# HKPolyU-UAV/FLVIS

Hardware: AMD Instinct MI355X
Metric: frames/sec/node (640×480 stereo+IMU) + ATE vs CPU ref, EuRoC MH_05 (higher is better)
Workload: dtype u8/f32 LK+GFTT, f64 geometry+BA

## Files before the change

### flvis_amd/csrc/capi.cpp

```cpp
#include <cmath>
#include <cstdint>
#include <cstdio>
#include <cstring>
#include <vector>

#include "../../include/flvis_hip.h"
#include "ctx.hpp"
#include "pipeline.hpp"

using namespace flvis;

void* flvis_ctx::scratch(const std::string& name, size_t bytes, bool zero_on_alloc) {
  Buf& b = bufs[name];
  if (b.bytes >= bytes && b.p) return b.p;
  if (b.p) {
    hipStreamSynchronize(stream);
    hipFree(b.p);
    b.p = nullptr;
    b.bytes = 0;
  }
  size_t want = (bytes + 255) / 256 * 256;
  if (hipMalloc(&b.p, want) != hipSuccess) {
    b.p = nullptr;
    return nullptr;
// ... 176 lines not shown
    total += pyr.stride[l] * n_img + 256;
    total = (total + 255) / 256 * 256;
  }
  uint8_t* base = (uint8_t*)ctx->scratch(name, total + 256);
  if (!base && L > 0) return ctx->fail(FLVIS_ERR_HIP, "pyramid scratch allocation failed");
  for (int l = 1; l <= L; l++) {
    pyr.lvl[l] = img_plain(base + off[l]);
    launch_pyr_down(ctx->stream, pyr.lvl[l - 1], pyr.w[l - 1], pyr.h[l - 1], pyr.pitch[l - 1], pyr.stride[l - 1],
                    pyr.lvl[l], pyr.pitch[l], pyr.stride[l], n_img, nullptr);
  }
  return FLVIS_OK;
}

int flvis_hip_lk_track(flvis_ctx* ctx, const uint8_t* d_prev, const uint8_t* d_next, int w, int h, int n_img,
                       const float* d_prev_pts, float* d_next_pts, uint8_t* d_status, const int* d_count, int nmax,
                       int max_level, int max_iter, double eps, int use_initial_flow) {
  CHECK_CTX(ctx);
  if (!d_prev || !d_next || !d_prev_pts || !d_next_pts || !d_status || !d_count || w < 32 || h < 32 || n_img <= 0 || nmax <= 0 ||
      max_level < 0)
    return ctx->fail(FLVIS_ERR_INVALID_ARG, "lk_track: bad args");
  int L = lk_levels(w, h, 31, max_level);
  if (L >= LK_MAX_LEVELS) L = LK_MAX_LEVELS - 1;
  PyrSel pp, pn;
  int rc = build_pyramid(ctx, "lk_pyr_prev", d_prev, w, h, n_img, L, pp);
  if (rc) return rc;
  rc = build_pyramid(ctx, "lk_pyr_next", d_next, w, h, n_img, L, pn);
  if (rc) return rc;
  LKParams prm;
  prm.max_iter = max_iter < 0 ? 0 : (max_iter > 100 ? 100 : max_iter);
  double e = eps < 0 ? 0 : (eps > 10 ? 10 : eps);
  prm.eps2 = e * e;
  prm.min_eig = 1e-4f;
  prm.use_initial = use_initial_flow ? 1 : 0;
  launch_lk_track(ctx->stream, pp, pn, d_prev_pts, d_next_pts, d_status, d_count, nmax, n_img, prm, nullptr);
  CHECK_LAUNCH(ctx, "lk_track");
  return FLVIS_OK;
}

int flvis_hip_rand_seed(flvis_ctx* ctx, uint32_t seed, int32_t* d_state35, int n_sets) {
  CHECK_CTX(ctx);
  if (!d_state35 || n_sets <= 0) return ctx->fail(FLVIS_ERR_INVALID_ARG, "rand_seed: bad args");
  std::vector<int> h((size_t)35 * n_sets);
  glibc_seed(seed, h.data());
  h[34] = 0;
  for (int s = 1; s < n_sets; s++) memcpy(&h[(size_t)35 * s], h.data(), sizeof(int) * 35);
  hipError_t e = hipMemcpyAsync(d_state35, h.data(), sizeof(int) * h.size(), hipMemcpyHostToDevice, ctx->stream);
  if (e == hipSuccess) e = hipStreamSynchronize(ctx->stream);
  if (e != hipSuccess) return ctx->hip_fail(e, "rand_seed");
  return FLVIS_OK;
}

int flvis_hip_stereo_depth(flvis_ctx* ctx, const flvis_cfg* cfg, const uint8_t* d_img0, const uint8_t* d_img1, int n_sets,
                           const float* d_pt2d_plane, const float* d_pt2d_undistort, const float* d_pt3d_w, const uint8_t* d_has_depth,
                           const int* d_count, int cap, const double* h_T_c_w7, float range, int32_t* d_rand_state35, double* d_pt3d_c,
                           uint8_t* d_mask_has_3d) {
  CHECK_CTX(ctx);
  if (!cfg || !d_img0 || !d_img1 || !d_pt2d_plane || !d_pt2d_undistort || !d_pt3d_w || !d_has_depth || !d_count || !h_T_c_w7 ||
      !d_rand_state35 || !d_pt3d_c || !d_mask_has_3d || n_sets <= 0 || cap <= 0)
    return ctx->fail(FLVIS_ERR_INVALID_ARG, "stereo_depth: bad args");
  if (cfg->cam_type == CAM_DEPTH) return ctx->fail(FLVIS_ERR_CONFIG, "stereo_depth: the rig has a depth camera (recover3DPts_c_FromDepthImg), no stereo pair");
  const int w = cfg->image_width, h = cfg->image_height;
  if (w < 32 || h < 32) return ctx->fail(FLVIS_ERR_CONFIG, "stereo_depth: image too small");
  if (cfg->P0[0] == 0.0 || cfg->P0[5] == 0.0 || cfg->P1[0] == 0.0)
    return ctx->fail(FLVIS_ERR_CONFIG, "stereo_depth: the configuration is not finalised (flvis_config_finalize: P0 / P1 are empty)");
  flvis_sd_cam cam;
  memcpy(cam.K1, cfg->cam1_intrinsics, 32);
  memcpy(cam.D1, cfg->cam1_distortion, 32);
  memcpy(cam.R1, cfg->R1, 72);
// ... 152 lines not shown
```

### flvis_amd/csrc/ctx.hpp

```cpp
#pragma once
#include <hip/hip_runtime.h>

#include <map>
#include <memory>
#include <string>

#include "img_kernels.hpp"

namespace flvis {
struct Pipeline;
}

struct flvis_ctx {
  int device = 0;
  hipStream_t stream = nullptr;
  bool own_stream = false;
  std::string err;

  struct Buf {
    void* p = nullptr;
    size_t bytes = 0;
  };
  std::map<std::string, Buf> bufs;
  flvis::Pipeline* pipe = nullptr;
  int voc_nodes = 0, voc_words = 0, voc_depth = 0;
  std::string orb_pattern;

  void* scratch(const std::string& name, size_t bytes, bool zero_on_alloc = false);
  int fail(int code, const std::string& msg) {
    err = msg;
    return code;
  }
  int hip_fail(hipError_t e, const char* what) {
    err = std::string(what) + ": " + hipGetErrorString(e);
    return -3;
  }
};

static inline int align_up(int v, int a) { return (v + a - 1) / a * a; }
```

### flvis_amd/csrc/img_kernels.hpp

```cpp
#pragma once
#include <hip/hip_runtime.h>
#include <stdint.h>

namespace flvis {

struct KJoin {
  const long long* wait[2];
  long long wait_seq[2];
  long long* sig;
  long long sig_seq;
  unsigned* sig_cnt;
  long long* err;
  const long long* post;
  long long post_seq;
};


struct ImgSel {
  const uint8_t* b[2];
  const int* cur;
  int flip;
  const uint8_t* const* ind;
  __device__ const uint8_t* ptr(int s, size_t stride) const {
    if (ind) return *ind + (size_t)s * stride;
    int k = cur ? (cur[s] ^ flip) : 0;
    return b[k] + (size_t)s * stride;
  }
};
static inline ImgSel img_plain(const uint8_t* p) { return ImgSel{{p, p}, nullptr, 0, nullptr}; }
static inline ImgSel img_indirect(const uint8_t* const* slot) { return ImgSel{{nullptr, nullptr}, nullptr, 0, slot}; }

constexpr int LK_MAX_LEVELS = 6;
struct PyrSel {
  ImgSel lvl[LK_MAX_LEVELS];
  int w[LK_MAX_LEVELS], h[LK_MAX_LEVELS], pitch[LK_MAX_LEVELS];
  size_t stride[LK_MAX_LEVELS];
  int levels;
  int bx[LK_MAX_LEVELS] = {}, by[LK_MAX_LEVELS] = {};
};
constexpr int LK_BORDER_X = 32, LK_BORDER_Y = 24;

struct LKParams {
  int max_iter;
  double eps2;
  float min_eig;
  int use_initial;
  unsigned long long* stats = nullptr;
  unsigned long long* stats_tc = nullptr;
  uint32_t* tc = nullptr;
  int tc_mode = 0, tc_cap = 0, tc_stride = 0;
  const int* tc_slot = nullptr;
  const long long* tc_tag = nullptr;
  int order = 0;
  int dbg_slot = 0;
};
int lk_tc_slot_dwords(int levels);
__device__ inline int lk_tc_lookup(const uint32_t* tc, int tc_cap, int tc_stride, int s, int slot, float px, float py, long long tag) {
  if (!tc || slot < 0 || slot >= tc_cap) return -1;
  const uint32_t* h = tc + ((size_t)s * tc_cap + slot) * tc_stride;
  if (h[0] != __float_as_uint(px) || h[1] != __float_as_uint(py) || *reinterpret_cast<const long long*>(h + 2) != tag) return -1;
  return slot | (int)((h[4] & 0x7fffu) << 16);
}

struct DemParams {
  int regionWidth, regionHeight, boundary_dis;
  unsigned max_region_feature_num;
};

struct GfttScratch {
  unsigned* maxenc;
  int* nkeys;
  unsigned long long* keys;
  int cap;
};

hipError_t img_kernels_init();
void launch_equalize_hist(hipStream_t st, ImgSel src, ImgSel dst, int w, int h, int spitch, int dpitch, size_t sstride,
                          size_t dstride, int S, unsigned* hist, uint8_t* lut, const int* active);
void launch_bgr_to_gray(hipStream_t st, const uint8_t* src, int channels, uint8_t* dst, size_t npixels);
void launch_copy_image(hipStream_t st, ImgSel src, ImgSel dst, int w, int h, int spitch, int dpitch, size_t sstride,
                       size_t dstride, int S, const int* active);
// ... 42 lines not shown
```

### flvis_amd/csrc/lk_kernel.hip

```cpp
#include "dev_common.hpp"
#include "img_kernels.hpp"

namespace flvis {

constexpr int LK_WIN = 31;
constexpr int LK_PS = 40;
constexpr int LK_PROWS = 34;
constexpr int LK_RM = 4;
constexpr int LK_RS = 52;
constexpr int LK_RROWS = 33 + 2 * LK_RM;
constexpr int LK_TC_HDR = 64;
constexpr int LK_TC_LVL = 64 * 24;

typedef short lk_s2 __attribute__((ext_vector_type(2)));
typedef __attribute__((address_space(1))) uint32_t lk_gu32;
typedef uint32_t lk_u4 __attribute__((ext_vector_type(4)));
__device__ __forceinline__ lk_s2 lk_as_s2(uint32_t v) { return __builtin_bit_cast(lk_s2, v); }

__device__ __forceinline__ bool lk_load_patch(const uint8_t* __restrict__ img, int w, int h, int pitch, int bx, int by, int X0, int Y0,
                                              int nrows, uint8_t* patch) {
  if (X0 >= -bx && Y0 >= -by && X0 + 39 < w + bx && Y0 + nrows <= h + by) {
    const lk_gu32* const base = (const lk_gu32*)(img + (ptrdiff_t)Y0 * pitch + (X0 & ~3));
    const int sh = X0 & 3;
    int r = (int)threadIdx.x / 9, k = (int)threadIdx.x - 9 * r;
// ... 58 lines not shown
    constexpr int N = LK_RROWS * 13, T = (N + 63) / 64;
    uint32_t v[T];
#pragma unroll
    for (int t = 0; t < T; t++) {
      const bool on = 64 * (t + 1) <= N || (int)threadIdx.x + 64 * t < N;
      v[t] = *(const lk_gu32*)(base + (on ? off : 0u));
      k += 12;
      const bool wrap = k >= 13;
      k = wrap ? k - 13 : k;
      off += (unsigned)(4 * pitch + 48) + (wrap ? (unsigned)(pitch - 52) : 0u);
    }
#pragma unroll
    for (int t = 0; t < T; t++) asm volatile("" : "+v"(v[t]));
#pragma unroll
    for (int t = 0; t < T; t++)
      if (64 * (t + 1) <= N || (int)threadIdx.x + 64 * t < N) *reinterpret_cast<uint32_t*>(region + 4 * ((int)threadIdx.x + 64 * t)) = v[t];
    return false;
  }
  for (int i = threadIdx.x; i < LK_RROWS * 13; i += 64) {
    int r = i / 13, k = i - r * 13;
    int Y = Y0 + r, X = X0 + 4 * k;
    uint32_t v;
    if (Y >= 0 && Y < h && X >= 0 && X + 3 < w) {
      v = *reinterpret_cast<const uint32_t*>(img + (size_t)Y * pitch + X);
    } else {
      const uint8_t* row = img + (size_t)reflect101c(Y, h) * pitch;
      uint32_t b0 = row[reflect101c(X, w)], b1 = row[reflect101c(X + 1, w)], b2 = row[reflect101c(X + 2, w)],
               b3 = row[reflect101c(X + 3, w)];
      v = b0 | (b1 << 8) | (b2 << 16) | (b3 << 24);
    }
    *reinterpret_cast<uint32_t*>(region + r * LK_RS + 4 * k) = v;
  }
  return true;
}

#define LK_PAIR(D, K)                                                                                              \
  ((((K)&3) == 3) ? __builtin_amdgcn_perm((D)[((K) >> 2) + 1], (D)[(K) >> 2], 0x0c040c03u)                         \
                  : __builtin_amdgcn_perm(0u, (D)[(K) >> 2], 0x0c000c00u | (uint32_t)((K)&3) | ((uint32_t)(((K)&3) + 1) << 16)))

__device__ __forceinline__ int lk_dot2_bias(lk_s2 a, lk_s2 b, int bias_uniform) {
  int r;
  asm("v_dot2_i32_i16 %0, %1, %2, %3" : "=v"(r) : "v"(a), "v"(b), "s"(bias_uniform));
  return r;
}
__device__ __forceinline__ void lk_wave_sum2_f32(int v1, int v2, float& f1, float& f2) {
  int a = v1 & 0xffff, b = v1 >> 16, c = v2 & 0xffff, d = v2 >> 16;
#define LK_STEP4(CTRL, RM)                                           \
  {                                                                  \
    const int ta = __builtin_amdgcn_update_dpp(0, a, CTRL, RM, 0xf, false); \
    const int tb = __builtin_amdgcn_update_dpp(0, b, CTRL, RM, 0xf, false); \
    const int tc = __builtin_amdgcn_update_dpp(0, c, CTRL, RM, 0xf, false); \
    const int td = __builtin_amdgcn_update_dpp(0, d, CTRL, RM, 0xf, false); \
    a += ta, b += tb, c += tc, d += td;                              \
  }
  LK_STEP4(0xB1, 0xf)
  LK_STEP4(0x4E, 0xf)
  LK_STEP4(0x141, 0xf)
  LK_STEP4(0x140, 0xf)
  LK_STEP4(0x142, 0xa)
  LK_STEP4(0x143, 0xc)
#undef LK_STEP4
  const float g1 = (float)__builtin_fma((double)b, 65536.0, (double)a), g2 = (float)__builtin_fma((double)d, 65536.0, (double)c);
  f1 = __builtin_bit_cast(float, __builtin_amdgcn_readlane(__builtin_bit_cast(int, g1), 63));
  f2 = __builtin_bit_cast(float, __builtin_amdgcn_readlane(__builtin_bit_cast(int, g2), 63));
}

// ... 183 lines not shown
#ifdef FLVIS_LK_UTIL
__device__ unsigned long long g_lk_wt[3][8][32768][2];
#define LK_UTIL_BEGIN const unsigned long long lk_t0_ = wall_clock64(); const unsigned lk_widx_ = (blockIdx.y * gridDim.x + blockIdx.x) & 32767u;
#define LK_UTIL_END(ROLE)                                                              \
  if (threadIdx.x == 0) {                                                              \
    unsigned long long* u_ = g_lk_wt[(ROLE) % 3][prm.dbg_slot & 7][lk_widx_];          \
    u_[0] = lk_t0_;                                                                    \
    u_[1] = wall_clock64();                                                            \
  }
#else
#define LK_UTIL_BEGIN
#define LK_UTIL_END(ROLE)
#endif
template <int ROLE>
__device__ __forceinline__ void lk_track_body(const PyrSel& prev, const PyrSel& next, const float* __restrict__ prev_pts,
                                              float* __restrict__ next_pts, uint8_t* __restrict__ status,
                                              const int* __restrict__ count, int nmax, const LKParams& prm,
                                              const int* __restrict__ active) {
  int s = blockIdx.y, bx = blockIdx.x;
  {
    const int G = gridDim.x, N = G * gridDim.y;
    if ((N & 7) == 0) {
      const int L = bx + G * s;
      const int Lp = (L & 7) * (N >> 3) + (L >> 3);
      s = Lp / G;
      bx = Lp - s * G;
    }
  }
  if (active && !active[s]) return;
  int n = count[s];
  if (n > nmax) n = nmax;
  if (bx >= n) return;
  LK_UTIL_BEGIN
  __shared__ __attribute__((aligned(16))) uint8_t patch[LK_RROWS * LK_RS + 12];
  const int lane = threadIdx.x;
  int kc_prev = 0, kc_next = 0;
#pragma unroll
  for (int l = LK_MAX_LEVELS - 1; l >= 0; l--) {
    if (l <= prev.levels && prev.lvl[l].cur) kc_prev = prev.lvl[l].cur[s];
    if (l <= next.levels && next.lvl[l].cur) kc_next = next.lvl[l].cur[s];
  }
  const uint8_t* const ind_prev0 = prev.lvl[0].ind ? *prev.lvl[0].ind : nullptr;
  const uint8_t* const ind_next0 = next.lvl[0].ind ? *next.lvl[0].ind : nullptr;
  const int r = lane >> 1;
  const int c0 = (lane & 1) * 16;
  const int W_BITS = 14;
  double eps2 = prm.eps2;
  if (ROLE == 1 || ROLE == 4) asm volatile("" : "+v"(eps2));
  const float FLT_SCALE = 1.f / (1 << 20);
  const float halfWin = (LK_WIN - 1) * 0.5f;

  for (int pb = bx; pb < n; pb += gridDim.x) {
    const int p = prm.order == 1 ? n - 1 - pb : pb;
    const size_t pi = ((size_t)s * nmax + p) * 2;
    const float ppx0 = prev_pts[pi], ppy0 = prev_pts[pi + 1];
    float nx = next_pts[pi], ny = next_pts[pi + 1];
    int st = 1;
    uint32_t* tc_ptr = nullptr;
    bool tc_store = false, tc_hit = false;
    uint32_t tc_mask = 0;
    if (ROLE == 2 && prm.tc_mode == 1) {
      if (p < prm.tc_cap) {
        tc_store = true;
        tc_ptr = prm.tc + ((size_t)s * prm.tc_cap + p) * prm.tc_stride;
      }
    } else if ((ROLE == 1 && prm.tc_mode == 2) || (ROLE == 4 && prm.tc_mode == 3)) {
      const int code = __builtin_amdgcn_readfirstlane(prm.tc_slot[(size_t)s * nmax + p]);
      if (code >= 0 && (code & 0xffff) < prm.tc_cap) {
        tc_ptr = prm.tc + ((size_t)s * prm.tc_cap + (code & 0xffff)) * prm.tc_stride;
        tc_hit = true;
        tc_mask = (uint32_t)code >> 16;
      } else if (ROLE == 4 && code <= -2 && -code - 2 < prm.tc_cap) {
        tc_ptr = prm.tc + ((size_t)s * prm.tc_cap + (-code - 2)) * prm.tc_stride;
        tc_store = true;
      }
    }
    lk_u4 pq[6] = {};
    int pq_level = -1;
    for (int level = prev.levels; level >= 0; level--) {
      const float sc = (float)(1. / (1 << level));
      float ppx = ppx0 * sc, ppy = ppy0 * sc;
      float npx, npy;
      if (level == prev.levels) {
        if (prm.use_initial) {
          npx = nx * sc;
          npy = ny * sc;
        } else {
          npx = ppx;
          npy = ppy;
        }
      } else {
        npx = nx * 2.f;
        npy = ny * 2.f;
      }
      nx = npx;
      ny = npy;
      const int W = prev.w[level], H = prev.h[level];
      ppx -= halfWin;
      ppy -= halfWin;
      const int ipx = (int)floorf(ppx), ipy = (int)floorf(ppy);
      if (ipx < -LK_WIN || ipx >= W || ipy < -LK_WIN || ipy >= H) {
        if (level == 0) st = 0;
        continue;
      }
      float a = ppx - (float)ipx, b = ppy - (float)ipy;
      int iw00 = __float2int_rn((1.f - a) * (1.f - b) * (float)(1 << W_BITS));
      int iw01 = __float2int_rn(a * (1.f - b) * (float)(1 << W_BITS));
      int iw10 = __float2int_rn((1.f - a) * b * (float)(1 << W_BITS));
      int iw11 = (1 << W_BITS) - iw00 - iw01 - iw10;

      lk_s2 tI[8], tX[8], tY[8];
      long long iA11, iA12, iA22;
      const bool cached = (ROLE == 1 || ROLE == 4) && tc_hit && ((tc_mask >> level) & 1u);
      constexpr bool kEarlyRegion = (ROLE == 1 || ROLE == 4) && FLVIS_LK_EARLY_REGION;
      int JW = 0, JH = 0;
      const uint8_t* Jimg = nullptr;
      if (kEarlyRegion) {
        JW = next.w[level], JH = next.h[level];
        Jimg = lk_level_ptr(next, level, s, kc_next, ind_next0);
      }
      bool region_ok = false;
      int RX0 = 0, RY0 = 0;
      if (cached) {
        if (prm.stats_tc && lane == 0) atomicAdd(&prm.stats_tc[0], 1ull);
        if (pq_level != level) {
          const lk_u4* src = reinterpret_cast<const lk_u4*>(tc_ptr + LK_TC_HDR + (size_t)level * LK_TC_LVL) + lane;
#pragma unroll
          for (int k = 0; k < 6; k++) pq[k] = __builtin_nontemporal_load(src + 64 * k);
        }
        if (kEarlyRegion) {
        {
          const int einx = (int)floorf(npx - halfWin), einy = (int)floorf(npy - halfWin);
          if (!(einx < -LK_WIN || einx >= JW || einy < -LK_WIN || einy >= JH)) {
            RX0 = (einx - LK_RM) & ~3;
            RY0 = einy - LK_RM;
            __syncthreads();
            const bool slow = lk_load_region(Jimg, JW, JH, next.pitch[level], next.bx[level], next.by[level], RX0, RY0, patch);
            __syncthreads();
            if (prm.stats_tc && slow && lane == 0) atomicAdd(&prm.stats_tc[2], 1ull);
            region_ok = true;
          }
        }
        }
        lk_u4 q[6];
#pragma unroll
        for (int k = 0; k < 6; k++) q[k] = pq[k];
        pq_level = -1;
        iA11 = (long long)(((unsigned long long)(uint32_t)__builtin_amdgcn_readlane((int)q[0].y, 63) << 32) | (uint32_t)__builtin_amdgcn_readlane((int)q[0].x, 63));
        iA12 = (long long)(((unsigned long long)(uint32_t)__builtin_amdgcn_readlane((int)q[0].w, 63) << 32) | (uint32_t)__builtin_amdgcn_readlane((int)q[0].z, 63));
        iA22 = (long long)(((unsigned long long)(uint32_t)__builtin_amdgcn_readlane((int)q[1].y, 63) << 32) | (uint32_t)__builtin_amdgcn_readlane((int)q[1].x, 63));
#pragma unroll
        for (int k = 0; k < 2; k++) {
          tI[4 * k + 0] = lk_as_s2(q[k].x); tI[4 * k + 1] = lk_as_s2(q[k].y);
          tI[4 * k + 2] = lk_as_s2(q[k].z); tI[4 * k + 3] = lk_as_s2(q[k].w);
          tX[4 * k + 0] = lk_as_s2(q[2 + k].x); tX[4 * k + 1] = lk_as_s2(q[2 + k].y);
          tX[4 * k + 2] = lk_as_s2(q[2 + k].z); tX[4 * k + 3] = lk_as_s2(q[2 + k].w);
          tY[4 * k + 0] = lk_as_s2(q[4 + k].x); tY[4 * k + 1] = lk_as_s2(q[4 + k].y);
          tY[4 * k + 2] = lk_as_s2(q[4 + k].z); tY[4 * k + 3] = lk_as_s2(q[4 + k].w);
        }
      } else if (ROLE == 1 || ROLE == 4) {
        LKTmpl T;
        lk_template_level_cold(lk_level_ptr(prev, level, s, kc_prev, ind_prev0), W, H, prev.pitch[level], prev.bx[level], prev.by[level], ipx, ipy, iw00,
                               iw01, iw10, iw11, patch, lane, &T);
#pragma unroll
        for (int k = 0; k < 8; k++) {
          tI[k] = lk_as_s2(T.w[k]);
          tX[k] = lk_as_s2(T.w[8 + k]);
          tY[k] = lk_as_s2(T.w[16 + k]);
        }
        iA11 = T.a11;
        iA12 = T.a12;
        iA22 = T.a22;
        if (ROLE == 4 && tc_store) {
          lk_tc_store_level(tc_ptr, level, lane, tI, tX, tY, iA11, iA12, iA22);
          tc_mask |= 1u << level;
        }
      } else {
        const bool slow = lk_template_level(lk_level_ptr(prev, level, s, kc_prev, ind_prev0), W, H, prev.pitch[level], prev.bx[level], prev.by[level], ipx,
                                            ipy, iw00, iw01, iw10, iw11, patch, lane, tI, tX, tY, iA11, iA12, iA22);
        if (prm.stats_tc && slow && lane == 0) atomicAdd(&prm.stats_tc[1], 1ull);
#ifndef FLVIS_LK_NO_TC_STORE
        if (ROLE == 2 && tc_store) {
          lk_tc_store_level(tc_ptr, level, lane, tI, tX, tY, iA11, iA12, iA22);
          tc_mask |= 1u << level;
        }
#endif
      }
      const float A11 = (float)iA11 * FLT_SCALE, A12 = (float)iA12 * FLT_SCALE, A22 = (float)iA22 * FLT_SCALE;
      float D = A11 * A22 - A12 * A12;
      const float minEig = __fdiv_rn(A22 + A11 - sqrtf((A11 - A22) * (A11 - A22) + 4.f * A12 * A12),
                                     (float)(2 * LK_WIN * LK_WIN));
      if (minEig < prm.min_eig || D < 1.1920929e-07f) {
        if (level == 0) st = 0;
        continue;
      }
      D = __fdiv_rn(1.f, D);
      npx -= halfWin;
      npy -= halfWin;
      float pdx = 0.f, pdy = 0.f;
      if (!kEarlyRegion) {
        JW = next.w[level], JH = next.h[level];
        Jimg = lk_level_ptr(next, level, s, kc_next, ind_next0);
      }
      int iters_run = 0;
      for (int j = 0; j < prm.max_iter; j++) {
        iters_run = j + 1;
        const int inx = (int)floorf(npx), iny = (int)floorf(npy);
        if (inx < -LK_WIN || inx >= JW || iny < -LK_WIN || iny >= JH) {
          if (level == 0) st = 0;
          break;
        }
        a = npx - (float)inx;
        b = npy - (float)iny;
        iw00 = __float2int_rn((1.f - a) * (1.f - b) * (float)(1 << W_BITS));
        iw01 = __float2int_rn(a * (1.f - b) * (float)(1 << W_BITS));
        iw10 = __float2int_rn((1.f - a) * b * (float)(1 << W_BITS));
        iw11 = (1 << W_BITS) - iw00 - iw01 - iw10;
        if (!region_ok || inx < RX0 || inx - RX0 > 15 || iny < RY0 || iny - RY0 > 2 * LK_RM) {
          RX0 = (inx - LK_RM) & ~3;
          RY0 = iny - LK_RM;
          __syncthreads();
          const bool slow = lk_load_region(Jimg, JW, JH, next.pitch[level], next.bx[level], next.by[level], RX0, RY0, patch);
          __syncthreads();
          if (prm.stats_tc && slow && lane == 0) atomicAdd(&prm.stats_tc[2], 1ull);
          region_ok = true;
        }
        int b1 = 0, b2 = 0;
        if (r < LK_WIN) {
          const int bx = inx - RX0 + c0, sh = bx & 3;
          const uint8_t* rp = patch + (iny - RY0 + r) * LK_RS + (bx & ~3);
          uint32_t e[2][5];
#pragma unroll
          for (int q = 0; q < 2; q++) {
            uint32_t dd[6];
#pragma unroll
            for (int k = 0; k < 6; k++) dd[k] = *reinterpret_cast<const uint32_t*>(rp + q * LK_RS + 4 * k);
#pragma unroll
            for (int k = 0; k < 5; k++) e[q][k] = __builtin_amdgcn_alignbyte(dd[k + 1], dd[k], sh);
          }
          const lk_s2 wT = lk_s2{(short)iw00, (short)iw01}, wB = lk_s2{(short)iw10, (short)iw11};
#pragma unroll
          for (int c2 = 0; c2 < 8; c2++) {
            int iv[2];
#pragma unroll
            for (int hh = 0; hh < 2; hh++) {
              const int c = 2 * c2 + hh;
              const uint32_t pt = LK_PAIR(e[0], c), pb = LK_PAIR(e[1], c);
              int acc = lk_dot2_bias(__builtin_bit_cast(lk_s2, pt), wT, 1 << (W_BITS - 5 - 1));
              acc = __builtin_amdgcn_sdot2(__builtin_bit_cast(lk_s2, pb), wB, acc, false);
              iv[hh] = acc >> (W_BITS - 5);
            }
            const lk_s2 ivp = __builtin_bit_cast(lk_s2, __builtin_amdgcn_perm((uint32_t)iv[1], (uint32_t)iv[0], 0x05040100u));
            const lk_s2 diff = ivp - tI[c2];
            b1 = __builtin_amdgcn_sdot2(diff, tX[c2], b1, false);
            b2 = __builtin_amdgcn_sdot2(diff, tY[c2], b2, false);
          }
        }
        float sb1, sb2;
        lk_wave_sum2_f32(b1, b2, sb1, sb2);
        const float fb1 = sb1 * FLT_SCALE, fb2 = sb2 * FLT_SCALE;
        const float ddx = (A12 * fb2 - A22 * fb1) * D;
        const float ddy = (A12 * fb1 - A11 * fb2) * D;
        npx += ddx;
        npy += ddy;
        nx = npx + halfWin;
        ny = npy + halfWin;
        if ((double)ddx * (double)ddx + (double)ddy * (double)ddy <= eps2) break;
        if (j > 0 && fabs((double)(ddx + pdx)) < 0.01 && fabs((double)(ddy + pdy)) < 0.01) {
          nx -= ddx * 0.5f;
          ny -= ddy * 0.5f;
          break;
        }
        pdx = ddx;
        pdy = ddy;
      }
      if (prm.stats && lane == 0) {
        atomicAdd(&prm.stats[2 * level], (unsigned long long)iters_run);
        atomicAdd(&prm.stats[2 * level + 1], 1ull);
      }
      if (st && level == 0) {
        const float fx = nx - halfWin, fy = ny - halfWin;
        const int inx = (int)floorf(fx), iny = (int)floorf(fy);
        if (inx < -LK_WIN || inx >= JW || iny < -LK_WIN || iny >= JH) st = 0;
      }
    }
    if (lane == 0) {
      next_pts[pi] = nx;
      next_pts[pi + 1] = ny;
      status[(size_t)s * nmax + p] = (uint8_t)st;
      if ((ROLE == 2 || ROLE == 4) && tc_store) {
        tc_ptr[0] = __float_as_uint(ppx0);
        tc_ptr[1] = __float_as_uint(ppy0);
        *reinterpret_cast<long long*>(tc_ptr + 2) = prm.tc_tag[s];
        tc_ptr[4] = tc_mask;
      }
    }
  }
  LK_UTIL_END(ROLE)
}
// ... 122 lines not shown
```

### flvis_amd/csrc/pipeline.cpp

```cpp
#include <algorithm>
#include <chrono>
#include <cmath>
#include <cstddef>
#include <cstdio>
#include <cstdlib>
#include <cstring>
#include <thread>
#include <limits>
#include <vector>

#include "../../include/flvis_hip.h"
#include "ctx.hpp"
#include "track_kernels.hpp"

namespace flvis {

constexpr int PROF_STAGES = 20;
static const char* kStageNames[PROF_STAGES] = {
    "imu_feed+frame_begin", "ingest(equalize)", "pyr_down(left)", "track_prepare", "lk_track(temporal)", "track_collect",
    "ransac_f", "ransac_pnp", "track_post+pose_lm", "reproj_filter", "gftt:eig_cand", "gftt:(merged)", "gftt:pick",
    "feature_dem+add_new", "depth_prepare", "lk_track(stereo)", "depth_innovate", "frame_end",
    "ba_worker(launch)", "frame(chain)"};

struct Lane {
// ... 1183 lines not shown
    PB(17, st);
    L->endf_valid = fold_signal(pl, L, L->ev_endf, p.kj);
    launch_frame_end(st, p);
    p.kj = KJoin{};
    PE(17, st);
    PE(19, st);
    if (prof)
      for (int i = 1; i < PROF_STAGES; i++)
        if (i != 17 && i != 19) {
          PB(i, st);
          PE(i, st);
        }
    if (!skipped) local_map_tail(nullptr, false);
    return;
  }
  const bool first_processed = pl->frames_fed == (long long)pl->cfg.skip_first_n_imgs;
  if (first_processed && L->idx > 0) hipStreamWaitEvent(st, pl->lanes[L->idx - 1]->ev_stagger, 0);
  PB(3, st);
  if (!head_prepare) launch_track_prepare(st, p);
  PE(3, st);
  if (!head_posts) join_wait(pl, L, st, L->ev_img);
  const bool r_in_place = !eq && aligned;
  ImgSel r0 = r_in_place ? in1 : img_plain(L->pyr1[0]);
  const int r0pitch = r_in_place ? w : pl->lpitch[0];
  const size_t r0stride = r_in_place ? (size_t)w * h : pl->lstride[0];
  PB(4, st);
  {
    PyrSel prev, next;
    fill_pyr(pl, prev, L->pyr0[0], L->pyr0[1], p.img_slot, 1, pl->levels_t);
    fill_pyr(pl, next, L->pyr0[0], L->pyr0[1], p.img_slot, 0, pl->levels_t);
    LKParams prm{30, 1e-3 * 1e-3, 1e-4f, 1};
    if (pl->lk_stats) prm.stats = reinterpret_cast<unsigned long long*>(p.counters) + 36;
    if (pl->lk_stats) prm.stats_tc = reinterpret_cast<unsigned long long*>(p.counters) + 61;
    if (L->tc) {
      prm.tc = L->tc;
      prm.tc_mode = 2;
      prm.tc_cap = p.tc_cap;
      prm.tc_stride = L->tc_stride;
      prm.tc_slot = p.lk_slot;
      prm.tc_tag = p.lk_tag;
    }
    prm.dbg_slot = (int)(pl->frames_fed & 7);
    launch_lk_track(st, prev, next, p.prev_pts, p.next_pts, p.lk_status, p.lk_count, NMAX, S, prm, p.act_track, pl->max_pts, 1);
  }
  PE(4, st);
  const int tpl_start = pl->tpl_start;
  auto templates_ahead = [&] {
    hipStream_t ts = L->tpl_stream;
    join_wait(pl, L, ts, tpl_start == 1 ? L->ev_lm : L->ev_tpl);
    PyrSel img;
    fill_pyr(pl, img, L->pyr0[0], L->pyr0[1], p.img_slot, 0, pl->levels_s);
    launch_lk_templates_ahead(ts, img, p.tpl_pts, p.tpl_count, NMAX, S, L->tc, p.tc_cap, L->tc_stride, p.tpl_tag, pl->max_pts);
    join_signal(pl, L, L->ev_tpl, ts);
  };
  const int chain_merge = pl->chain_merge;
  const bool merge_collect = (chain_merge & 2) && !(p.tpl_ahead && tpl_start == 0);
  PB(5, st);
  if (!merge_collect) launch_track_collect(st, p);
  PE(5, st);
  if (p.tpl_ahead && tpl_start == 0) {
    join_signal(pl, L, L->ev_tpl, st);
    templates_ahead();
  }
  if (first_processed && pl->lanes.size() > 1) hipEventRecord(L->ev_stagger, st);
  PB(6, st);
  const bool rf_signals = fold_signal(pl, L, L->ev_lm, p.kj);
// ... 50 lines not shown
                     p.new_xy, p.n_new, NEW_MAX, &dem_kj);
  const bool an_signals = fold_signal(pl, L, L->ev_lm, p.kj);
  const bool merge_seeds = (chain_merge & 1) != 0;
  if (!merge_seeds) {
    launch_add_new(st, p);
    p.kj = KJoin{};
  }
  PE(13, st);
  PB(14, st);
  const bool ds_signals = an_signals;
  const bool seeds_post = fold_post(pl, L, L->ev_det, p.kj);
  if (p.tpl_ahead && !fold_wait(pl, L, L->ev_tpl, p.kj, 0)) join_wait(pl, L, st, L->ev_tpl);
  if (merge_seeds) launch_add_new_seeds(st, p);
  else launch_depth_seeds(st, p);
  p.kj = KJoin{};
  PE(14, st);
  if (!ds_signals) join_signal(pl, L, L->ev_lm, st);
  join_wait(pl, L, ds, L->ev_lm);
  launch_depth_triangulate(ds, p);
  join_signal(pl, L, L->ev_tri, ds);
  if (!seeds_post) join_wait(pl, L, st, L->ev_det);
  PB(15, st);
  if (!depth_cam) {
    PyrSel prev, next;
    fill_pyr(pl, prev, L->pyr0[0], L->pyr0[1], p.img_slot, 0, pl->levels_s);
    fill_pyr(pl, next, L->pyr1, nullptr, nullptr, 0, pl->levels_s);
    next.lvl[0] = r0;
    next.pitch[0] = r0pitch;
    next.stride[0] = r0stride;
    if (r_in_place) next.bx[0] = next.by[0] = 0;
    LKParams prm{30, 1e-3 * 1e-3, 1e-4f, 1};
    if (pl->lk_stats) prm.stats = reinterpret_cast<unsigned long long*>(p.counters) + 48;
    if (pl->lk_stats) prm.stats_tc = reinterpret_cast<unsigned long long*>(p.counters) + 61;
    if (L->tc) {
      prm.tc = L->tc;
      prm.tc_mode = p.tpl_ahead ? 3 : 1;
      prm.tc_cap = p.tc_cap;
      prm.tc_stride = L->tc_stride;
      prm.tc_tag = p.lk_tag;
      prm.tc_slot = p.lk_slot;
    }
    prm.dbg_slot = (int)(pl->frames_fed & 7);
    prm.order = 1;
    launch_lk_track(st, prev, next, p.prev_pts, p.next_pts, p.lk_status, p.lk_count, NMAX, S, prm, p.det_mode, pl->max_pts,
                    L->tc && p.tpl_ahead ? 4 : 2);
  }
  PE(15, st);
  const bool inn_waits = fold_wait(pl, L, L->ev_tri, p.kj, 0);
  if (!inn_waits) join_wait(pl, L, st, L->ev_tri);
  PB(16, st);
  launch_depth_innovate(st, p);
  p.kj = KJoin{};
  PE(16, st);
  if (with_local_map) {
    const long long D = lane_backpressure_depth(pl, L);
    for (int k = 0; k < pl->nba_lane; k++) {
      const long long j = L->ba_launches - 1 - D - k;
      if (j >= 0 && L->ba_launches - j <= Lane::BAQ) {
        if (!(k < 2 && fold_wait(pl, L, L->ev_ba_done[j % Lane::BAQ], p.kj, k))) join_wait(pl, L, st, L->ev_ba_done[j % Lane::BAQ]);
      }
    }
  }
  PB(17, st);
  L->endf_valid = fold_signal(pl, L, L->ev_endf, p.kj);
  launch_frame_end(st, p);
  p.kj = KJoin{};
// ... 988 lines not shown
```

### include/flvis_hip.h

```cpp
#ifndef FLVIS_HIP_H
#define FLVIS_HIP_H

#include <stddef.h>
#include <stdint.h>

#ifdef __cplusplus
extern "C" {
#endif

typedef struct flvis_ctx flvis_ctx;

typedef enum flvis_status {
  FLVIS_OK = 0,
  FLVIS_ERR_INVALID_ARG = -1,
  FLVIS_ERR_NO_DEVICE = -2,
  FLVIS_ERR_HIP = -3,
  FLVIS_ERR_CAPACITY = -4,
  FLVIS_ERR_CONFIG = -5
} flvis_status;

const char* flvis_version(void);

#define FLVIS_STREAM_NEW ((void*)(intptr_t)-1)
int flvis_hip_create(int device, void* hip_stream, flvis_ctx** out);
// ... 191 lines not shown
typedef struct flvis_keyframe {
  int64_t frame_id;
  int8_t command;
  double stamp;
  flvis_image img0, img1;
  int32_t lm_count;
  const int64_t* lm_id;
  const double* lm_2d;
  const double* lm_3d;
  double T_c_w[7];
} flvis_keyframe;
int flvis_get_keyframe_msg(flvis_ctx* ctx, int stream, int cap, flvis_keyframe* kf, int64_t* h_lm_id, double* h_lm_2d,
                           double* h_lm_3d, uint8_t* h_img0, uint8_t* h_img1);
int flvis_get_correction(flvis_ctx* ctx, int stream, int cap, int64_t* frame_id, double* T_c_w7, int* lm_count,
                         int64_t* h_lm_id, double* h_lm_3d, int* lm_outlier_count, int64_t* h_outlier_id);

int flvis_correction_feed(flvis_ctx* ctx, int stream, int64_t frame_id, const double* T_c_w7, int lm_count,
                          const int64_t* h_lm_id, const double* h_lm_3d, int lm_outlier_count,
                          const int64_t* h_lm_outlier_id);
int flvis_get_pose_records(flvis_ctx* ctx, int stream, int cap, double* h_rows8);
int flvis_get_trajectory(flvis_ctx* ctx, int stream, int first_frame, int n_frames, double* h_rows9);
int flvis_write_trajectory(flvis_ctx* ctx, int stream, int first_frame, int n_frames, const char* path, int format,
                           double min_dt);
int flvis_write_imu_trajectory(const double* h_rows11, int n, const char* path, double min_dt, int append);
int flvis_write_imu_trajectory_run(const double* h_rows11, int n, const char* path, double min_dt, int append, double t_first);
int flvis_reset_streams(flvis_ctx* ctx, int n, const int* streams);
int flvis_reset_streams_rigs(flvis_ctx* ctx, int n, const int* streams, const flvis_cfg* cfgs);
int flvis_local_map_reset(flvis_ctx* ctx, int n, const int* streams);
int flvis_get_counters(flvis_ctx* ctx, int64_t* h_counters3);
int flvis_get_counters_n(flvis_ctx* ctx, int n, int64_t* h_counters);
int flvis_get_local_map_counts(flvis_ctx* ctx, int64_t* h_keyframes, int64_t* h_ba_runs);
int flvis_debug_stage_poses(flvis_ctx* ctx, int stream, double* h_out21);
int flvis_debug_lk_stats(flvis_ctx* ctx, int enable);
int flvis_debug_pyramid(flvis_ctx* ctx, const uint8_t* d_src, int w, int h, int n_img, int levels, int bx, int by, int ingest, uint8_t* d_out,
                        size_t out_bytes);
int flvis_hip_debug_corner_response(flvis_ctx* ctx, const uint8_t* d_img, int w, int h, int n_img, int variant, int rows,
                                    uint32_t* h_max_bits, int* h_nkeys, uint64_t* h_keys, int key_cap);
int flvis_hip_debug_sqrt_check(flvis_ctx* ctx, uint32_t first_bits, uint32_t n, uint64_t* h_mismatches);
int flvis_debug_counters(flvis_ctx* ctx, int64_t* h_counters64);

int flvis_ba_push_keyframe(flvis_ctx* ctx, int stream, int64_t frame_id, const double* T_c_w7, int lm_count,
                           const int64_t* h_lm_id, const double* h_lm_2d, const double* h_lm_3d, int cap,
                           int64_t* out_frame_id, double* out_T_c_w7, int* out_lm_count, int64_t* out_lm_id,
                           double* out_lm_3d, int* out_outlier_count, int64_t* out_outlier_id);

int flvis_set_imu_factor(flvis_ctx* ctx, int enable, double sigma_gyro);
int flvis_set_imu_factor_accel(flvis_ctx* ctx, double sigma_acc);
int flvis_get_keyframe_imu_pos(flvis_ctx* ctx, int stream, double* dp3, double* va3);
int flvis_ba_push_keyframe_imu_pos(flvis_ctx* ctx, int stream, int64_t frame_id, const double* T_c_w7, const double* imu_dq_wxyz,
                                   double imu_dt, const double* imu_dp3, const double* imu_va3, int lm_count, const int64_t* h_lm_id,
                                   const double* h_lm_2d, const double* h_lm_3d, int out_cap, int64_t* out_frame_id, double* out_T_c_w7,
                                   int* out_lm_count, int64_t* out_lm_id, double* out_lm_3d, int* out_outlier_count,
                                   int64_t* out_outlier_id);
int flvis_get_keyframe_imu(flvis_ctx* ctx, int stream, double* dq_wxyz, double* dt);
int flvis_ba_push_keyframe_imu(flvis_ctx* ctx, int stream, int64_t frame_id, const double* T_c_w7, const double* imu_dq_wxyz,
                               double imu_dt, int lm_count, const int64_t* h_lm_id, const double* h_lm_2d, const double* h_lm_3d,
                               int cap, int64_t* out_frame_id, double* out_T_c_w7, int* out_lm_count, int64_t* out_lm_id,
                               double* out_lm_3d, int* out_outlier_count, int64_t* out_outlier_id);

typedef struct flvis_lc_params {
  int lcKFStart, lcKFDist, lcKFMaxDist, lcKFLast, lcNKFClosest, minPts;
  double ratioMax, ratioRansac, minScore;
} flvis_lc_params;
typedef struct flvis_lc_event {
  int64_t kf_prev, kf_curr;
  int candidate;
// ... 83 lines not shown
```

Baseline: 62080.

## Prefetch next pyramid level's LK region and templates into LDS asynchronously

During the first LK iteration at each pyramid level, the kernel predicts the next level's search window and issues global_load_lds DMA copies of that image region into a second LDS buffer (double buffering). Cached template blocks for the next level are also prefetched into LDS. The next level then uses the staged region if the prediction holds, and skips the synchronous region load and the nontemporal global template loads. This increases LDS use, which may lower occupancy, and adds vmcnt drains and speculative loads that are wasted when the prediction misses. A debug API for counting prefetch hits is added as well.

```diff
diff --git a/flvis_amd/csrc/capi.cpp b/flvis_amd/csrc/capi.cpp
--- a/flvis_amd/csrc/capi.cpp
+++ b/flvis_amd/csrc/capi.cpp
@@ -232,8 +232,29 @@
   prm.eps2 = e * e;
   prm.min_eig = 1e-4f;
   prm.use_initial = use_initial_flow ? 1 : 0;
+  if (ctx->lk_pf_stats) prm.stats_pf = ctx->lk_pf_stats;
   launch_lk_track(ctx->stream, pp, pn, d_prev_pts, d_next_pts, d_status, d_count, nmax, n_img, prm, nullptr);
   CHECK_LAUNCH(ctx, "lk_track");
+  return FLVIS_OK;
+}
+
+int flvis_debug_lk_prefetch(flvis_ctx* ctx, int enable, int64_t* h_out12) {
+  CHECK_CTX(ctx);
+  const size_t bytes = sizeof(unsigned long long) * 12;
+  hipError_t e = hipDeviceSynchronize();
+  if (e != hipSuccess) return ctx->hip_fail(e, "lk_prefetch");
+  if (h_out12) {
+    for (int i = 0; i < 12; i++) h_out12[i] = 0;
+    if (ctx->lk_pf_stats && (e = hipMemcpy(h_out12, ctx->lk_pf_stats, bytes, hipMemcpyDeviceToHost)) != hipSuccess)
+      return ctx->hip_fail(e, "lk_prefetch");
+  }
+  ctx->lk_pf_stats = nullptr;
+  if (enable) {
+    unsigned long long* p = (unsigned long long*)ctx->scratch("lk_pf_stats", bytes);
+    if (!p) return ctx->fail(FLVIS_ERR_HIP, "lk_prefetch: allocation failed");
+    if ((e = hipMemset(p, 0, bytes)) != hipSuccess) return ctx->hip_fail(e, "lk_prefetch");
+    ctx->lk_pf_stats = p;
+  }
   return FLVIS_OK;
 }
 
diff --git a/flvis_amd/csrc/ctx.hpp b/flvis_amd/csrc/ctx.hpp
--- a/flvis_amd/csrc/ctx.hpp
+++ b/flvis_amd/csrc/ctx.hpp
@@ -24,6 +24,7 @@
   std::map<std::string, Buf> bufs;
   flvis::Pipeline* pipe = nullptr;
   int voc_nodes = 0, voc_words = 0, voc_depth = 0;
+  unsigned long long* lk_pf_stats = nullptr;
   std::string orb_pattern;
 
   void* scratch(const std::string& name, size_t bytes, bool zero_on_alloc = false);
diff --git a/flvis_amd/csrc/img_kernels.hpp b/flvis_amd/csrc/img_kernels.hpp
--- a/flvis_amd/csrc/img_kernels.hpp
+++ b/flvis_amd/csrc/img_kernels.hpp
@@ -47,6 +47,7 @@
   int use_initial;
   unsigned long long* stats = nullptr;
   unsigned long long* stats_tc = nullptr;
+  unsigned long long* stats_pf = nullptr;
   uint32_t* tc = nullptr;
   int tc_mode = 0, tc_cap = 0, tc_stride = 0;
   const int* tc_slot = nullptr;
diff --git a/flvis_amd/csrc/lk_kernel.hip b/flvis_amd/csrc/lk_kernel.hip
--- a/flvis_amd/csrc/lk_kernel.hip
+++ b/flvis_amd/csrc/lk_kernel.hip
@@ -114,6 +114,39 @@
     *reinterpret_cast<uint32_t*>(region + r * LK_RS + 4 * k) = v;
   }
   return true;
+}
+
+typedef __attribute__((address_space(3))) uint32_t lk_lu32;
+__device__ __forceinline__ void lk_dma_drain() { asm volatile("s_waitcnt vmcnt(0)" ::: "memory"); }
+
+__device__ __forceinline__ void lk_prefetch_region(const uint8_t* __restrict__ img, int pitch, int X0, int Y0, uint8_t* region) {
+  const __attribute__((address_space(1))) uint8_t* const base = (const __attribute__((address_space(1))) uint8_t*)(img + (ptrdiff_t)Y0 * pitch + X0);
+  lk_lu32* const dst = (lk_lu32*)region;
+  constexpr int N = LK_RROWS * 13, T = (N + 63) / 64;
+  static_assert(N >= 64 && (T - 1) * 64 <= N, "full trips, then the last 64 items");
+  int l = (int)threadIdx.x;
+  asm volatile("" : "+v"(l));
+  int r = (l * 0x13b2) >> 16, k = l - 13 * r;
+  unsigned off = (unsigned)(r * pitch + 4 * k);
+#pragma unroll
+  for (int t = 0; t < T - 1; t++) {
+    __builtin_amdgcn_global_load_lds((const lk_gu32*)(base + off), dst + 64 * t, 4, 0, 0);
+    k += 12;
+    const bool wrap = k >= 13;
+    k = wrap ? k - 13 : k;
+    off += (unsigned)(4 * pitch + 48) + (wrap ? (unsigned)(pitch - 52) : 0u);
+  }
+  const int i = l + (N - 64);
+  r = (i * 0x13b2) >> 16;
+  k = i - 13 * r;
+  __builtin_amdgcn_global_load_lds((const lk_gu32*)(base + (unsigned)(r * pitch + 4 * k)), dst + (N - 64), 4, 0, 0);
+}
+
+__device__ __forceinline__ void lk_prefetch_templates(const uint32_t* tc_ptr, int level, int lane, uint8_t* tbuf) {
+  typedef __attribute__((address_space(1))) lk_u4 lk_gu4;
+  const lk_gu4* const src = (const lk_gu4*)(tc_ptr + LK_TC_HDR + (size_t)level * LK_TC_LVL) + lane;
+#pragma unroll
+  for (int k = 0; k < 6; k++) __builtin_amdgcn_global_load_lds(src + 64 * k, (lk_lu32*)(tbuf + 1024 * k), 16, 0, 2);
 }
 
 #define LK_PAIR(D, K)                                                                                              \
@@ -363,7 +396,12 @@
   if (n > nmax) n = nmax;
   if (bx >= n) return;
   LK_UTIL_BEGIN
-  __shared__ __attribute__((aligned(16))) uint8_t patch[LK_RROWS * LK_RS + 12];
+  constexpr int LK_RBUF = LK_RROWS * LK_RS + 12, LK_TBUF = ROLE == 1 ? 4 * LK_TC_LVL : 0;
+  static_assert(LK_RBUF % 16 == 0, "16-byte aligned buffers");
+  __shared__ __attribute__((aligned(16))) uint8_t lds[LK_TBUF + 2 * LK_RBUF];
+  uint8_t* const tbuf = lds;
+  uint8_t* const rbuf = lds + LK_TBUF;
+  int pf = 0;
   const int lane = threadIdx.x;
   int kc_prev = 0, kc_next = 0;
 #pragma unroll
@@ -406,9 +444,13 @@
         tc_store = true;
       }
     }
-    lk_u4 pq[6] = {};
-    int pq_level = -1;
+    pf &= 1;
     for (int level = prev.levels; level >= 0; level--) {
+      const int pfl = __builtin_amdgcn_readfirstlane(pf);
+      const bool spec_here = (pfl & 2) != 0, tq_here = ROLE == 1 && (pfl & 4) != 0;
+      if (pfl & 6) lk_dma_drain();
+      pf = pfl & 1;
+      uint8_t* const patch = rbuf + (pfl & 1) * LK_RBUF;
       const float sc = (float)(1. / (1 << level));
       float ppx = ppx0 * sc, ppy = ppy0 * sc;
       float npx, npy;
@@ -432,6 +474,7 @@
       const int ipx = (int)floorf(ppx), ipy = (int)floorf(ppy);
       if (ipx < -LK_WIN || ipx >= W || ipy < -LK_WIN || ipy >= H) {
         if (level == 0) st = 0;
+        if (prm.stats_pf && tq_here && lane == 0) atomicAdd(&prm.stats_pf[3], 1ull);
         continue;
       }
       float a = ppx - (float)ipx, b = ppy - (float)ipy;
@@ -454,12 +497,17 @@
       int RX0 = 0, RY0 = 0;
       if (cached) {
         if (prm.stats_tc && lane == 0) atomicAdd(&prm.stats_tc[0], 1ull);
-        if (pq_level != level) {
+        lk_u4 q[6];
+        if (tq_here) {
+#pragma unroll
+          for (int k = 0; k < 6; k++) q[k] = *reinterpret_cast<const lk_u4*>(tbuf + 1024 * k + 16 * lane);
+          if (prm.stats_pf && lane == 0) atomicAdd(&prm.stats_pf[2], 1ull);
+        } else {
           const lk_u4* src = reinterpret_cast<const lk_u4*>(tc_ptr + LK_TC_HDR + (size_t)level * LK_TC_LVL) + lane;
 #pragma unroll
-          for (int k = 0; k < 6; k++) pq[k] = __builtin_nontemporal_load(src + 64 * k);
-        }
-        if (kEarlyRegion) {
+          for (int k = 0; k < 6; k++) q[k] = __builtin_nontemporal_load(src + 64 * k);
+        }
+        if (kEarlyRegion && !spec_here) {
         {
           const int einx = (int)floorf(npx - halfWin), einy = (int)floorf(npy - halfWin);
           if (!(einx < -LK_WIN || einx >= JW || einy < -LK_WIN || einy >= JH)) {
@@ -473,10 +521,6 @@
           }
         }
         }
-        lk_u4 q[6];
-#pragma unroll
-        for (int k = 0; k < 6; k++) q[k] = pq[k];
-        pq_level = -1;
         iA11 = (long long)(((unsigned long long)(uint32_t)__builtin_amdgcn_readlane((int)q[0].y, 63) << 32) | (uint32_t)__builtin_amdgcn_readlane((int)q[0].x, 63));
         iA12 = (long long)(((unsigned long long)(uint32_t)__builtin_amdgcn_readlane((int)q[0].w, 63) << 32) | (uint32_t)__builtin_amdgcn_readlane((int)q[0].z, 63));
         iA22 = (long long)(((unsigned long long)(uint32_t)__builtin_amdgcn_readlane((int)q[1].y, 63) << 32) | (uint32_t)__builtin_amdgcn_readlane((int)q[1].x, 63));
@@ -533,6 +577,16 @@
         JW = next.w[level], JH = next.h[level];
         Jimg = lk_level_ptr(next, level, s, kc_next, ind_next0);
       }
+      if (spec_here) {
+        pf ^= 1;
+        RX0 = ((int)((unsigned)pfl << 14) >> 17) * 4;
+        RY0 = pfl >> 18;
+        region_ok = true;
+      }
+#pragma unroll
+      for (int k = 0; k < 8; k++) asm volatile("" ::"v"(tI[k]), "v"(tX[k]), "v"(tY[k]));
+      const int cur = (pfl ^ (pfl >> 1)) & 1;
+      uint8_t* const region = rbuf + cur * LK_RBUF;
       int iters_run = 0;
       for (int j = 0; j < prm.max_iter; j++) {
         iters_run = j + 1;
@@ -547,11 +601,17 @@
         iw01 = __float2int_rn(a * (1.f - b) * (float)(1 << W_BITS));
         iw10 = __float2int_rn((1.f - a) * b * (float)(1 << W_BITS));
         iw11 = (1 << W_BITS) - iw00 - iw01 - iw10;
-        if (!region_ok || inx < RX0 || inx - RX0 > 15 || iny < RY0 || iny - RY0 > 2 * LK_RM) {
+        bool stage = !region_ok || inx < RX0 || inx - RX0 > 15 || iny < RY0 || iny - RY0 > 2 * LK_RM;
+        if (j == 0 && spec_here) {
+          const int ox = (inx - LK_RM) & ~3, oy = iny - LK_RM;
+          stage = stage || ox < -next.bx[level] || oy < -next.by[level] || ox + 51 >= JW + next.bx[level] || oy + LK_RROWS > JH + next.by[level];
+          if (prm.stats_pf && lane == 0) atomicAdd(&prm.stats_pf[stage ? 1 : 0], 1ull);
+        }
+        if (stage) {
           RX0 = (inx - LK_RM) & ~3;
           RY0 = iny - LK_RM;
           __syncthreads();
-          const bool slow = lk_load_region(Jimg, JW, JH, next.pitch[level], next.bx[level], next.by[level], RX0, RY0, patch);
+          const bool slow = lk_load_region(Jimg, JW, JH, next.pitch[level], next.bx[level], next.by[level], RX0, RY0, region);
           __syncthreads();
           if (prm.stats_tc && slow && lane == 0) atomicAdd(&prm.stats_tc[2], 1ull);
           region_ok = true;
@@ -559,7 +619,7 @@
         int b1 = 0, b2 = 0;
         if (r < LK_WIN) {
           const int bx = inx - RX0 + c0, sh = bx & 3;
-          const uint8_t* rp = patch + (iny - RY0 + r) * LK_RS + (bx & ~3);
+          const uint8_t* rp = region + (iny - RY0 + r) * LK_RS + (bx & ~3);
           uint32_t e[2][5];
 #pragma unroll
           for (int q = 0; q < 2; q++) {
@@ -596,6 +656,24 @@
         npy += ddy;
         nx = npx + halfWin;
         ny = npy + halfWin;
+        if (j == 0 && level > 0) {
+          const int nl = level - 1;
+          const int einx = __builtin_amdgcn_readfirstlane((int)floorf(nx * 2.f - halfWin)),
+                    einy = __builtin_amdgcn_readfirstlane((int)floorf(ny * 2.f - halfWin));
+          const int w1 = next.w[nl], h1 = next.h[nl], bx1 = next.bx[nl], by1 = next.by[nl];
+          if (einx >= -LK_WIN && einx < w1 && einy >= -LK_WIN && einy < h1) {
+            const int X0 = (einx - LK_RM) & ~3, Y0 = einy - LK_RM;
+            if (X0 >= -bx1 && Y0 >= -by1 && X0 + 51 < w1 + bx1 && Y0 + LK_RROWS <= h1 + by1 && X0 >= -65536 && X0 < 65536 && Y0 >= -8192 &&
+                Y0 < 8192) {
+              lk_prefetch_region(lk_level_ptr(next, nl, s, kc_next, ind_next0), next.pitch[nl], X0, Y0, rbuf + (cur ^ 1) * LK_RBUF);
+              pf |= (int)(2u | (((unsigned)(X0 >> 2) & 0x7fffu) << 3) | ((unsigned)Y0 << 18));
+            }
+          }
+          if (ROLE == 1 && tc_hit && ((tc_mask >> nl) & 1u)) {
+            lk_prefetch_templates(tc_ptr, nl, lane, tbuf);
+            pf |= 4;
+          }
+        }
         if ((double)ddx * (double)ddx + (double)ddy * (double)ddy <= eps2) break;
         if (j > 0 && fabs((double)(ddx + pdx)) < 0.01 && fabs((double)(ddy + pdy)) < 0.01) {
           nx -= ddx * 0.5f;
diff --git a/flvis_amd/csrc/pipeline.cpp b/flvis_amd/csrc/pipeline.cpp
--- a/flvis_amd/csrc/pipeline.cpp
+++ b/flvis_amd/csrc/pipeline.cpp
@@ -1239,6 +1239,7 @@
     LKParams prm{30, 1e-3 * 1e-3, 1e-4f, 1};
     if (pl->lk_stats) prm.stats = reinterpret_cast<unsigned long long*>(p.counters) + 36;
     if (pl->lk_stats) prm.stats_tc = reinterpret_cast<unsigned long long*>(p.counters) + 61;
+    if (ctx->lk_pf_stats) prm.stats_pf = ctx->lk_pf_stats + 4;
     if (L->tc) {
       prm.tc = L->tc;
       prm.tc_mode = 2;
@@ -1355,6 +1356,7 @@
     LKParams prm{30, 1e-3 * 1e-3, 1e-4f, 1};
     if (pl->lk_stats) prm.stats = reinterpret_cast<unsigned long long*>(p.counters) + 48;
     if (pl->lk_stats) prm.stats_tc = reinterpret_cast<unsigned long long*>(p.counters) + 61;
+    if (ctx->lk_pf_stats) prm.stats_pf = ctx->lk_pf_stats + 8;
     if (L->tc) {
       prm.tc = L->tc;
       prm.tc_mode = p.tpl_ahead ? 3 : 1;
diff --git a/include/flvis_hip.h b/include/flvis_hip.h
--- a/include/flvis_hip.h
+++ b/include/flvis_hip.h
@@ -247,6 +247,7 @@
 int flvis_get_local_map_counts(flvis_ctx* ctx, int64_t* h_keyframes, int64_t* h_ba_runs);
 int flvis_debug_stage_poses(flvis_ctx* ctx, int stream, double* h_out21);
 int flvis_debug_lk_stats(flvis_ctx* ctx, int enable);
+int flvis_debug_lk_prefetch(flvis_ctx* ctx, int enable, int64_t* h_out12);
 int flvis_debug_pyramid(flvis_ctx* ctx, const uint8_t* d_src, int w, int h, int n_img, int levels, int bx, int by, int ingest, uint8_t* d_out,
                         size_t out_bytes);
 int flvis_hip_debug_corner_response(flvis_ctx* ctx, const uint8_t* d_img, int w, int h, int n_img, int variant, int rows,
```

New measurement: 60530. 2.5% lower.
